# Enderdead/Pytorch_Quantize_impls

Hardware: AMD Instinct MI355X
Metric: XNOR-popcount GEMM TOPS (LinearBin 4096x4096 forward, batch 4096 per GPU) (higher is better)
Workload: dtype fp4-e2m1 (+-1 exact) MFMA, fp32 accumulate, fp32 in/out; 1 GPU; c2: LinearBin(4096, 4096).train().forward(x) on fp32 +-1 activations = sign+pack(x) + sign+pack(W) + packed GEMM, timed through the module (autograd node included); batch_per_gpu=4096, in_features=4096, out_features=4096, global_batch=4096, parallelism=batch-shard x1, no collective, gemm_impl=mfma, detect_mode=verify, float_split=f16x2

## Files before the change

include/qt_hip.h:

```cpp
#ifndef QT_HIP_H
#define QT_HIP_H

#include <stdint.h>

#ifdef __cplusplus
extern "C" {
#endif

typedef void* qt_stream_t;

typedef enum qt_status {
    QT_OK = 0,
    QT_ERR_INVALID_ARG = -1,
    QT_ERR_ALIGNMENT = -2,
    QT_ERR_LAUNCH = -3,
    QT_ERR_UNSUPPORTED = -4,
    QT_ERR_NO_DEVICE = -5
} qt_status;

int qt_version(void);
const char* qt_strerror(int status);
const char* qt_target_arch(void);
int qt_device_info(char* name, int cap);

// ... 82 lines not shown
int qt_tern_gemm(const uint32_t* Xs, int64_t ldxp, const uint32_t* Wmask, const uint32_t* Wsign,
                 int64_t ldwp, const float* bias, float* Y, int64_t ldy, int64_t M, int64_t N,
                 int64_t K, qt_stream_t stream);


int qt_sign_pack_nib_f32(const float* x, int64_t ldx, uint32_t* nib_plane, int64_t ldp,
                         int64_t rows, int64_t K, qt_stream_t stream);

int qt_ternary_pack_nib_f32(const float* x, int64_t ldx, uint32_t* nib_plane, int64_t ldp,
                            int64_t rows, int64_t K, qt_stream_t stream);

int qt_sign0_pack_nib_f32(const float* x, int64_t ldx, uint32_t* nib_plane, int64_t ldp, int64_t rows, int64_t K,
                          qt_stream_t stream);

int qt_pack_pair_nib_f32(const float* x, int64_t ldx, uint32_t* x_plane, int64_t ldxp, int64_t rows_x,
                         const float* w, int64_t ldw, uint32_t* w_plane, int64_t ldwp, int64_t rows_w,
                         int64_t K, int w_ternary, qt_stream_t stream);

int qt_nib_gemm_describe(int64_t M, int64_t N, int64_t K, int64_t ldxp, int64_t ldwp, char* out, int cap);

int qt_nib_gemm(const uint32_t* Xn, int64_t ldxp, const uint32_t* Wn, int64_t ldwp,
                const float* bias, float* Y, int64_t ldy, int64_t M, int64_t N, int64_t K,
                qt_stream_t stream);


int qt_dorefa_codes_i8(const float* x, int64_t ldx, int8_t* codes, int64_t ldc_bytes, float* y_f32,
                       int64_t ldy, int64_t rows, int64_t K, int bit_width, int32_t* overflow,
                       qt_stream_t stream);

int qt_bn_eval_device_f32(const float* x, int64_t ldx, const float* weight, const float* bias, const float* bn_stats, float* y,
                          int64_t ldy, int64_t rows, int64_t C, qt_stream_t stream);

int qt_affine_dorefa_codes_i8(const float* x, int64_t ldx, const float* alpha, const float* beta,
                              const float* res_f32, int64_t ldr, const float* res_alpha, const float* res_beta,
                              const int8_t* res_codes, int64_t ldrc_bytes, float res_scale, int relu, int8_t* codes,
                              int64_t ldc_bytes, float* y_f32, int64_t ldy, int64_t rows, int64_t C, int bit_width,
                              int32_t* overflow, const float* bn_stats, const float* res_bn_stats, qt_stream_t stream);

int qt_affine_dorefa_codes_halo_i8(const float* x, int64_t ldx, const float* alpha, const float* beta,
                                   const float* res_f32, int64_t ldr, const float* res_alpha, const float* res_beta,
                                   const int8_t* res_codes, int64_t ldrc_bytes, float res_scale, int relu, int8_t* codes,
                                   int64_t ldc_bytes, int64_t N, int64_t H, int64_t W, int64_t C, int bit_width,
                                   int32_t* overflow, const float* bn_stats, const float* res_bn_stats, int64_t out_halo_h,
                                   int64_t out_halo_w, qt_stream_t stream);

int qt_codes_to_f32(const int8_t* codes, int64_t ld_bytes, int64_t N, int64_t H, int64_t W, int64_t halo_h, int64_t halo_w,
// ... 257 lines not shown
```

pytorch_quantize_impls_amd/_lib.py:

```python
from __future__ import annotations

import ctypes
import os
import re
import threading
from collections import Counter

_HERE = os.path.dirname(os.path.abspath(__file__))
LIB_PATH = os.environ.get("QT_HIP_LIB") or os.path.join(_HERE, "lib", "libqt_hip.so")
HEADER_PATH = os.path.normpath(os.path.join(_HERE, "..", "include", "qt_hip.h"))


class QtLibraryError(RuntimeError):
    """libqt_hip.so could not be loaded (not built, wrong arch, missing symbol)."""


class QtStatusError(RuntimeError):
    """A C-ABI entry point returned a negative qt_status."""


_c_i64 = ctypes.c_int64
_c_p = ctypes.c_void_p
_c_int = ctypes.c_int
_c_f32 = ctypes.c_float
# ... 39 lines not shown
    "qt_ternary_pack_nib_f32": (_c_int, [_c_p, _c_i64, _c_p, _c_i64, _c_i64, _c_i64, _c_p]),
    "qt_sign0_pack_nib_f32": (_c_int, [_c_p, _c_i64, _c_p, _c_i64, _c_i64, _c_i64, _c_p]),
    "qt_pack_pair_nib_f32": (_c_int, [_c_p, _c_i64, _c_p, _c_i64, _c_i64, _c_p, _c_i64, _c_p, _c_i64, _c_i64, _c_i64,
                                      _c_int, _c_p]),
    "qt_wgrad_pack_grad_f32": (_c_int, [_c_p, _c_i64, _c_i64, _c_i64, _c_i64, _c_i64, _c_i64, _c_i64, _c_i64, _c_i64, _c_p,
                                        _c_i64, _c_p]),
    "qt_wgrad_pack_act_f32": (_c_int, [_c_p, _c_i64, _c_i64, _c_i64, _c_i64, _c_i64, _c_i64, _c_i64, _c_i64, _c_i64, _c_i64,
                                       _c_i64, _c_i64, _c_f32, _c_p, _c_i64, _c_i64, _c_p]),
    "qt_bf16_gemm_taps": (_c_int, [_c_p, _c_i64, _c_p, _c_i64, _c_p, _c_i64, _c_i64, _c_i64, _c_i64, _c_i64, _c_i64, _c_i64,
                                   _c_i64, _c_i64, _c_i64, _c_p]),
    "qt_wgrad_reduce_f32": (_c_int, [_c_p, _c_i64, _c_i64, _c_i64, _c_i64, _c_i64, _c_i64, _c_p, _c_f32, _c_f32, _c_int, _c_p,
                                     _c_p]),
    "qt_wgrad_pm_pack_grad_f32": (_c_int, [_c_p] + [_c_i64] * 11 + [_c_p, _c_p]),
    "qt_wgrad_pm_pack_grad_bias_f32": (_c_int, [_c_p] + [_c_i64] * 10 + [_c_p, _c_p, _c_p]),
    "qt_wgrad_pm_bias_reduce_f32": (_c_int, [_c_p, _c_i64, _c_i64, _c_i64, _c_int, _c_p, _c_p]),
    "qt_wgrad_pm_pack_act_f32": (_c_int, [_c_p] + [_c_i64] * 13 + [_c_f32, _c_p, _c_p]),
    "qt_wgrad_pm_pack_act_s2d_f32": (_c_int, [_c_p] + [_c_i64] * 17 + [_c_p, _c_p]),
    "qt_wgrad_pm_pack_act_s2d_f16x2": (_c_int, [_c_p] + [_c_i64] * 17 + [_c_p, _c_p, _c_p]),
    "qt_wgrad_pm_pack_grad_f16x2": (_c_int, [_c_p] + [_c_i64] * 11 + [_c_p, _c_p, _c_p, _c_p]),
    "qt_wgrad_pm_pack_act_f16": (_c_int, [_c_p] + [_c_i64] * 13 + [_c_f32, _c_p, _c_p]),
    "qt_wgrad_pm_f16": (_c_int, [_c_p, _c_p, _c_p] + [_c_i64] * 7 + [_c_p]),
    "qt_wgrad_pm_f32": (_c_int, [_c_p, _c_p, _c_p] + [_c_i64] * 7 + [_c_p]),
    "qt_wgrad_pm_reduce_f32": (_c_int, [_c_p] + [_c_i64] * 6 + [_c_p, _c_f32, _c_f32, _c_p, _c_int, _c_p] + [_c_i64] * 4 + [_c_p]),
    "qt_nib_gemm_describe": (_c_int, [_c_i64, _c_i64, _c_i64, _c_i64, _c_i64, ctypes.c_char_p, _c_int]),
    "qt_nib_gemm": (_c_int, [_c_p, _c_i64, _c_p, _c_i64, _c_p, _c_p, _c_i64, _c_i64, _c_i64,
                             _c_i64, _c_p]),
    "qt_bits_to_nib": (_c_int, [_c_p, _c_p, _c_i64, _c_p, _c_i64, _c_i64, _c_i64, _c_p]),
    "qt_pack_conv_weight_codes_i8": (_c_int, [_c_p] + [_c_i64] * 8 + [_c_int, _c_p, _c_i64, _c_p]),
    "qt_dorefa_codes_i8": (_c_int, [_c_p, _c_i64, _c_p, _c_i64, _c_p, _c_i64, _c_i64, _c_i64, _c_int, _c_p, _c_p]),
    "qt_bn_eval_device_f32": (_c_int, [_c_p, _c_i64, _c_p, _c_p, _c_p, _c_p, _c_i64, _c_i64, _c_i64, _c_p]),
    "qt_affine_dorefa_codes_i8": (_c_int, [_c_p, _c_i64, _c_p, _c_p, _c_p, _c_i64, _c_p, _c_p, _c_p, _c_i64, _c_f32,
                                           _c_int, _c_p, _c_i64, _c_p, _c_i64, _c_i64, _c_i64, _c_int, _c_p, _c_p, _c_p, _c_p]),
    "qt_affine_dorefa_codes_halo_i8": (_c_int, [_c_p, _c_i64, _c_p, _c_p, _c_p, _c_i64, _c_p, _c_p, _c_p, _c_i64, _c_f32,
                                                _c_int, _c_p, _c_i64, _c_i64, _c_i64, _c_i64, _c_i64, _c_int, _c_p, _c_p, _c_p,
                                                _c_i64, _c_i64, _c_p]),
    "qt_codes_to_f32": (_c_int, [_c_p] + [_c_i64] * 7 + [_c_f32, _c_p, _c_i64, _c_p, _c_i64, _c_p]),
    "qt_weight_codes_i8": (_c_int, [_c_p, _c_i64, _c_p, _c_i64, _c_i64, _c_i64, _c_int, _c_p]),
    "qt_i8_gemm": (_c_int, [_c_p, _c_i64, _c_p, _c_i64, _c_p, _c_f32, _c_p, _c_i64, _c_p, _c_i64, _c_i64,
                            _c_i64, _c_i64, _c_p]),
    "qt_pool_affine_sign_pack_nhwc": (_c_int, [_c_p, _c_i64, _c_i64, _c_i64, _c_i64, _c_i64, _c_i64, _c_p, _c_p,
                                               _c_p, _c_i64, _c_int, _c_p]),
    "qt_pool_affine_sign_pack_nib_nhwc": (_c_int, [_c_p, _c_i64, _c_i64, _c_i64, _c_i64, _c_i64, _c_i64, _c_p, _c_p,
                                                   _c_p, _c_i64, _c_p, _c_i64, _c_int, _c_p]),
    "qt_bf16x3_pack_f32": (_c_int, [_c_p, _c_i64, _c_p, _c_p, _c_i64, _c_i64, _c_i64, _c_int, _c_p]),
    "qt_bf16x3_s2d_pack_f32": (_c_int, [_c_p, _c_i64, _c_i64, _c_i64, _c_i64, _c_p, _c_i64] + [_c_i64] * 7 + [_c_p]),
    "qt_bf16x6_pack_f32": (_c_int, [_c_p, _c_i64, _c_p, _c_i64, _c_i64, _c_i64, _c_int, _c_p]),
# ... 142 lines not shown
```

pytorch_quantize_impls_amd/csrc/mfma_gemm.hip:

```cpp

#include <cstdio>
#include "mfma_gemm_kernel.h"

namespace {

int check_common(const void* Xn, int64_t ldxp, const void* Wn, int64_t ldwp, const float* Y, int64_t ldy,
                 int64_t M, int64_t N, int64_t K, int64_t kwords) {
    if (M < 0 || N < 0 || K < 0) return QT_ERR_INVALID_ARG;
    if (M == 0 || N == 0) return 1;
    if (!Y || ldy < N) return QT_ERR_INVALID_ARG;
    if (M > INT32_MAX || N > INT32_MAX || K > INT32_MAX) return QT_ERR_UNSUPPORTED;
    if (K > 0 && (!Xn || !Wn)) return QT_ERR_INVALID_ARG;
    if (ldxp < kwords || ldwp < kwords) return QT_ERR_INVALID_ARG;
    if ((ldxp & 3) || (ldwp & 3)) return QT_ERR_ALIGNMENT;
    if (K > 0 && (!qt_aligned16(Xn) || !qt_aligned16(Wn))) return QT_ERR_ALIGNMENT;
    return QT_OK;
}

template <class E>
int dispatch_gemm(int variant, const uint32_t* Xn, int64_t ldxp, const uint32_t* Wn, int64_t ldwp,
                  const float* bias, float scale, const float* scale_dev, float* Y, int64_t ldy, int64_t M,
                  int64_t N, int64_t K, qt_stream_t stream) {
    const bool pipe_ok = !(ldxp & 31) && !(ldwp & 31) && M * ldxp * 4 < (1ll << 31) &&
                         N * ldwp * 4 < (1ll << 31);
// ... 82 lines not shown
                                                            uint32_t* __restrict__ oa, int64_t ldpa, int64_t rowsa,
                                                            const float* __restrict__ xb, int64_t ldb,
                                                            uint32_t* __restrict__ ob, int64_t ldpb, int64_t rowsb,
                                                            int64_t K) {
    const int64_t ta = rowsa * ldpa * 2, total = ta + rowsb * ldpb * 2;
    const int64_t k4 = K / 4;
    for (int64_t s = (int64_t)blockIdx.x * blockDim.x + threadIdx.x; s < total;
         s += (int64_t)gridDim.x * blockDim.x) {
        const bool second = s >= ta;
        const int64_t t = second ? s - ta : s;
        const int64_t spr = (second ? ldpb : ldpa) * 2;
        const int64_t row = t / spr, slot = t - row * spr;
        uint32_t h = 0;
        if (slot < k4) {
            const float4 v = *reinterpret_cast<const float4*>((second ? xb + row * ldb : xa + row * lda) + slot * 4);
            h = second ? (EncW::nib(v.x) | (EncW::nib(v.y) << 4) | (EncW::nib(v.z) << 8) | (EncW::nib(v.w) << 12))
                       : (NibSign::nib(v.x) | (NibSign::nib(v.y) << 4) | (NibSign::nib(v.z) << 8) | (NibSign::nib(v.w) << 12));
        }
        const uint32_t other = __shfl_xor(h, 1);
        if ((threadIdx.x & 1) == 0) (second ? ob + row * ldpb : oa + row * ldpa)[slot >> 1] = h | (other << 16);
    }
}

template <class Enc>
__global__ __launch_bounds__(256) void nib_pack_scalar_kernel(const float* __restrict__ x, int64_t ldx,
                                                              uint32_t* __restrict__ out, int64_t ldp,
                                                              int64_t rows, int64_t K) {
    const int64_t total = rows * ldp;
    for (int64_t i = (int64_t)blockIdx.x * blockDim.x + threadIdx.x; i < total;
         i += (int64_t)gridDim.x * blockDim.x) {
        const int64_t row = i / ldp, w = i - row * ldp;
        uint32_t word = 0;
#pragma unroll
        for (int e = 0; e < 8; ++e) {
            const int64_t k = w * 8 + e;
            if (k < K) word |= Enc::nib(x[row * ldx + k]) << (4 * e);
        }
        out[i] = word;
    }
}

__global__ __launch_bounds__(256) void bits_to_nib_kernel(const uint32_t* __restrict__ sign,
                                                          const uint32_t* __restrict__ mask,
                                                          int64_t ldb, uint32_t* __restrict__ out,
                                                          int64_t ldn, int64_t rows, int64_t K) {
    const int64_t groups_per_row = ldn / 4;
// ... 108 lines not shown
                         int w_ternary, qt_stream_t stream) {
    if (rows_x < 0 || rows_w < 0 || K < 0 || ldx < K || ldw < K) return QT_ERR_INVALID_ARG;
    const bool vec = rows_x > 0 && rows_w > 0 && K > 0 && (K % 4 == 0) && (ldx % 4 == 0) && (ldw % 4 == 0) &&
                     qt_aligned16(x) && qt_aligned16(w) && x && w && x_plane && w_plane;
    if (!vec) {
        const int rc = launch_nib_pack<NibSign>(x, ldx, x_plane, ldxp, rows_x, K, stream);
        if (rc != QT_OK) return rc;
        return w_ternary ? launch_nib_pack<NibTernary>(w, ldw, w_plane, ldwp, rows_w, K, stream)
                         : launch_nib_pack<NibSign>(w, ldw, w_plane, ldwp, rows_w, K, stream);
    }
    const int64_t kw = (K + 7) / 8;
    if (ldxp < kw || ldwp < kw || (ldxp & 3) || (ldwp & 3) || !qt_aligned16(x_plane) || !qt_aligned16(w_plane))
        return QT_ERR_ALIGNMENT;
    const int grid = qt_stream_grid(((rows_x * ldxp + rows_w * ldwp) * 2 + 255) / 256);
    if (w_ternary)
        hipLaunchKernelGGL((nib_pack_pair_kernel<NibTernary>), dim3(grid), dim3(256), 0, (hipStream_t)stream, x, ldx,
                           x_plane, ldxp, rows_x, w, ldw, w_plane, ldwp, rows_w, K);
    else
        hipLaunchKernelGGL((nib_pack_pair_kernel<NibSign>), dim3(grid), dim3(256), 0, (hipStream_t)stream, x, ldx,
                           x_plane, ldxp, rows_x, w, ldw, w_plane, ldwp, rows_w, K);
    return qt_check_launch();
}

int qt_nib_gemm_variant(int variant, const uint32_t* Xn, int64_t ldxp, const uint32_t* Wn,
                        int64_t ldwp, const float* bias, float* Y, int64_t ldy, int64_t M, int64_t N,
                        int64_t K, qt_stream_t stream) {
    const int rc = check_common(Xn, ldxp, Wn, ldwp, Y, ldy, M, N, K, (K + 7) / 8);
    if (rc != QT_OK) return rc > 0 ? QT_OK : rc;
    if (K >= (1 << 24)) return QT_ERR_UNSUPPORTED;
    return dispatch_gemm<ElemFp4>(variant, Xn, ldxp, Wn, ldwp, bias, 1.0f, nullptr, Y, ldy, M, N, K, stream);
}

int qt_nib_gemm_describe(int64_t M, int64_t N, int64_t K, int64_t ldxp, int64_t ldwp, char* out, int cap) {
    if (!out || cap < 2 || M <= 0 || N <= 0 || K < 0) return QT_ERR_INVALID_ARG;
    const bool pipe_ok = !(ldxp & 31) && !(ldwp & 31) && M * ldxp * 4 < (1ll << 31) && N * ldwp * 4 < (1ll << 31);
    const int tn = pick_tile_n_gemm(M, N);
    const char* cfg;
    if (pipe_ok && M <= 256 && !((ldxp | ldwp) & 127)) cfg = "64x64, 512-byte stages, pipe=1";
    else if (pipe_ok && M <= 512 && !((ldxp | ldwp) & 63)) cfg = "128x64, 256-byte stages, pipe=1";
    else if (pipe_ok && tn == 256) cfg = "256x256, pipe=2 (ping-pong)";
    else if (pipe_ok && tn == 192) cfg = prefer_384_rows(M, N) ? "384x192, pipe=2 (ping-pong)" : "256x192, pipe=2 (ping-pong)";
    else if (pipe_ok && tn == 128) cfg = "256x128, pipe=2 (ping-pong)";
    else if (pipe_ok) cfg = "256x64, pipe=1";
    else cfg = tn == 256 ? "256x256, pipe=0" : tn == 192 ? "256x192, pipe=0" : tn == 128 ? "256x128, pipe=0" : "256x64, pipe=0";
    snprintf(out, (size_t)cap, "mfma_gemm_kernel<ElemFp4, %s>", cfg);
    return QT_OK;
}

int qt_nib_gemm(const uint32_t* Xn, int64_t ldxp, const uint32_t* Wn, int64_t ldwp, const float* bias,
                float* Y, int64_t ldy, int64_t M, int64_t N, int64_t K, qt_stream_t stream) {
    return qt_nib_gemm_variant(0, Xn, ldxp, Wn, ldwp, bias, Y, ldy, M, N, K, stream);
}

int qt_bf16_gemm(const uint32_t* Xh, int64_t ldxp, const uint32_t* Wh, int64_t ldwp, const float* bias,
                 float* Y, int64_t ldy, int64_t M, int64_t N, int64_t K, qt_stream_t stream) {
    const int rc = check_common(Xh, ldxp, Wh, ldwp, Y, ldy, M, N, K, (K + 1) / 2);
    if (rc != QT_OK) return rc > 0 ? QT_OK : rc;
    return dispatch_gemm<ElemBf16>(0, Xh, ldxp, Wh, ldwp, bias, 1.0f, nullptr, Y, ldy, M, N, K, stream);
}

int qt_f16_gemm(const uint32_t* Xh, int64_t ldxp, const uint32_t* Wh, int64_t ldwp, const float* bias, float scale,
                const float* scale_dev, float* Y, int64_t ldy, int64_t M, int64_t N, int64_t K, qt_stream_t stream) {
    const int rc = check_common(Xh, ldxp, Wh, ldwp, Y, ldy, M, N, K, (K + 1) / 2);
    if (rc != QT_OK) return rc > 0 ? QT_OK : rc;
    return dispatch_gemm<ElemF16>(0, Xh, ldxp, Wh, ldwp, bias, scale, scale_dev, Y, ldy, M, N, K, stream);
}

int qt_bf16_gemm_taps(const uint32_t* Xh, int64_t ldxp, const uint32_t* Wh, int64_t ldwp, float* Y, int64_t ldy,
                      int64_t M, int64_t N, int64_t K, int64_t tap_rows, int64_t tap_cols, int64_t nslice,
// ... 344 lines not shown
```

pytorch_quantize_impls_amd/csrc/mfma_gemm_kernel.h:

```cpp
#pragma once
#include <cstdlib>
#include <type_traits>
#include "qt_common.h"
#include "pp_common.h"

namespace {

__device__ __attribute__((aligned(16))) const unsigned char zero16_storage[16] = {0};


struct ConvArgs {
    int H, W, Ho, Wo, kh, kw, sh, sw, ph, pw, dh, dw;
    int cpp;
    int kbytes;
    unsigned magic_cpp, magic_kw;
    int sh_hw = -1, sh_w = -1;
    int z_nslice = 0, z_kw = 1;
    long long z_kslice_bytes = 0, z_w_copy_bytes = 0, z_w_row_bytes = 0, z_y_stride = 0;
};

struct EpiArgs {
    const float* alpha = nullptr;
    const float* beta = nullptr;
    int mode = 0;
    int relu = 0;
    float levels = 0.0f;
    float rscale = 0.0f;
    const float* res_f32 = nullptr;
    const float* ralpha = nullptr;
    const float* rbeta = nullptr;
    const int8_t* res_codes = nullptr;
    int64_t ldr = 0, ldrc = 0;
    int32_t* overflow = nullptr;
    int ohy = 0, ohx = 0, rhy = 0, rhx = 0;
    int d2s_cout = 0;
    const float* thr = nullptr;
    const float* bn_stats = nullptr;
    unsigned long long magic_hw = 0, magic_w = 0;
    const float* tap_rho = nullptr;
    int tap_ksteps = 0, ntaps = 0;
    const float* row_A = nullptr;
    int aH = 0, aW = 0, aph = 0, apw = 0;
};

__device__ __forceinline__ uint32_t spread8(uint32_t b) {
    uint32_t t = b & 0xFFu;
    t = (t | (t << 12)) & 0x000F000Fu;
    t = (t | (t << 6)) & 0x03030303u;
    t = (t | (t << 3)) & 0x11111111u;
    return t;
}

__device__ __forceinline__ void zero_halo_border(void* plane, int cpp, int64_t nimg, int H, int W, int hy, int hx,
                                                 int zb, int nzb) {
    const int Hp = H + 2 * hy, Wp = W + 2 * hx;
    const int top = hy * Wp, side = 2 * hx * H, per_img = 2 * top + side;
    const int64_t total = nimg * per_img * cpp;
    uint4* Q = reinterpret_cast<uint4*>(plane);
    for (int64_t t = (int64_t)zb * blockDim.x + threadIdx.x; t < total; t += (int64_t)nzb * blockDim.x) {
        const int64_t bp = t / cpp;
        const int c = (int)(t - bp * cpp);
        const int64_t n = bp / per_img;
        const int b = (int)(bp - n * per_img);
        int pix;
        if (b < top) pix = b;
// ... 54 lines not shown
        typedef _Float16 h8 __attribute__((ext_vector_type(8)));
        h8 av, bv;
        __builtin_memcpy(&av, &a, 16);
        __builtin_memcpy(&bv, &b, 16);
        return __builtin_amdgcn_mfma_f32_32x32x16_f16(av, bv, c, 0, 0, 0);
    }
    __device__ __forceinline__ static float out(float v, float scale, float bias) { return v * scale + bias; }
};

struct ElemFp4Taps : ElemFp4 {
    static constexpr bool TAPS = true;
    __device__ __forceinline__ static float out(float v, float scale, float bias) { return v * scale + bias; }
};
struct ElemF16Taps : ElemF16 {
    static constexpr bool TAPS = true;
};
struct ElemFp4TapsRows : ElemFp4Taps {
    static constexpr bool ROWS = true;
};
struct ElemFp4T : ElemFp4 {
    static constexpr bool SWAPT = true;
    __device__ __forceinline__ static acc_t mfma(const uint4& a, const uint4& b, acc_t c) { return ElemFp4::mfma(b, a, c); }
};
template <class E, class = void> struct elem_swapt : std::false_type {};
template <class E> struct elem_swapt<E, std::void_t<decltype(E::SWAPT)>> : std::bool_constant<E::SWAPT> {};
template <class E, class = void> struct elem_rows : std::false_type {};
template <class E> struct elem_rows<E, std::void_t<decltype(E::ROWS)>> : std::bool_constant<E::ROWS> {};

template <class E_, int WM_, int WN_, int TMW_, int TNW_, int PIPE_, int ABL_ = 0, int SB_ = 128, int CONV_ = 0, int OCC_ = 1>
struct GemmCfg {
    using E = E_;
    static constexpr bool CONV = CONV_ != 0, VALID = CONV_ == 2;
    static constexpr int WM = WM_, WN = WN_, TMW = TMW_, TNW = TNW_, PIPE = PIPE_, ABL = ABL_;
    static constexpr int STAGE_BYTES = SB_, KK = SB_ / 32;
    static constexpr int ROWS_PER_PIECE = 1024 / SB_;
    static constexpr int CHUNKS = SB_ / 16;
    static constexpr int NWAVES = WM * WN, NTHREADS = NWAVES * 64;
    static constexpr int TM = WM * TMW * 32, TN = WN * TNW * 32;
    static constexpr int X_STAGE = TM * STAGE_BYTES, W_STAGE = TN * STAGE_BYTES;
    static constexpr int BUF = X_STAGE + W_STAGE;
    static constexpr int NBUF = PIPE_ == 2 ? 4 : (PIPE_ >= 3 ? PIPE_ : 2);
    static constexpr int LDS_FIXED = NBUF * BUF + 64;
    static constexpr int LDS_BYTES = LDS_FIXED;
    static_assert(PIPE_ != 2 || (SB_ == 64 && NWAVES == 8), "ping-pong: 64-byte stages, two waves per SIMD");
    static constexpr int WAVES_PER_SIMD = OCC_ * ((NWAVES + 3) / 4);
    static_assert(TM % (ROWS_PER_PIECE * NWAVES) == 0 && (TN % (ROWS_PER_PIECE * NWAVES) == 0 || PIPE_ >= 1),
// ... 19 lines not shown
        const int gx = (N + C::TN - 1) / C::TN, gy = (M + C::TM - 1) / C::TM;
        const int ntiles = gx * gy, per_xcd = (ntiles + 7) >> 3;
        const int b = blockIdx.x;
        if constexpr (C::CONV) {
            if (b >= 8 * per_xcd) {
                const int zs = epi.d2s_cout ? 2 : 1;
                zero_halo_border(Y, (int)(epi.mode == 2 ? ldy / 16 : ldy / 4), (int64_t)M / (cg.Ho * cg.Wo), zs * cg.Ho,
                                 zs * cg.Wo, epi.ohy, epi.ohx, b - 8 * per_xcd, (int)gridDim.x - 8 * per_xcd);
                return;
            }
        }
        const int o = (b & 7) * per_xcd + (b >> 3);
        if (o >= ntiles) return;
        if ((gx & 7) == 0 && (gy & 3) == 0) {
            const int st = o >> 5, in_st = o & 31, sgx = gx >> 3;
            tile_m = (st / sgx) * 4 + (in_st >> 3);
            tile_n = (st % sgx) * 8 + (in_st & 7);
        } else {
            tile_m = o / gx;
            tile_n = o - tile_m * gx;
        }
    }
    const int m0 = tile_m * C::TM, n0 = tile_n * C::TN;

    const int64_t ldx_b = ldx * 4, ldw_b = ldw * 4;
    const unsigned char* Xb = reinterpret_cast<const unsigned char*>(X);
    const unsigned char* Wb = reinterpret_cast<const unsigned char*>(W);
    if constexpr (!C::CONV && (std::is_same<E, ElemBf16>::value || std::is_same<E, ElemI8>::value)) {
        if (cg.z_nslice > 0) {
            const int z = blockIdx.y, slice = z / cg.H, tap = z - slice * cg.H;
            const int tr = tap / cg.z_kw, tc = tap - tr * cg.z_kw;
            Xb += (int64_t)slice * cg.z_kslice_bytes;
            Wb += (int64_t)slice * cg.z_kslice_bytes + (int64_t)tc * cg.z_w_copy_bytes + (int64_t)tr * cg.z_w_row_bytes;
            Y += ((int64_t)tap * cg.z_nslice + slice) * cg.z_y_stride;
        }
    }

    acc_t acc[C::TMW][C::TNW];
    constexpr bool SWAPT = elem_swapt<E>::value;
    if constexpr (SWAPT) {
#pragma unroll
        for (int b = 0; b < C::TNW; ++b) {
            const int nb = n0 + (wave_n * C::TNW + b) * 32 + 16 * lhalf;
#pragma unroll
            for (int r4 = 0; r4 < 4; ++r4) {
                float4 t = make_float4(0, 0, 0, 0);
// ... 381 lines not shown
            dma_operand(Xb, ldx_b, m0, M, smem, C::TM, 0);
            dma_operand(Wb, ldw_b, n0, N, smem + C::X_STAGE, C::TN, 0);
        }
        __syncthreads();
        for (int s = 0; s < nstages; ++s) {
            const int buf = s & 1;
            const unsigned char* xs = smem + buf * BUF;
            const unsigned char* ws = xs + C::X_STAGE;
            uint4 xf[KK][C::TMW], wf[KK][C::TNW];
#pragma unroll
            for (int kk = 0; kk < KK; ++kk) read_frags(xs, ws, kk, xf[kk], wf[kk]);
            if (s + 1 < nstages) {
                dma_operand(Xb, ldx_b, m0, M, smem + (buf ^ 1) * BUF, C::TM, s + 1);
                dma_operand(Wb, ldw_b, n0, N, smem + (buf ^ 1) * BUF + C::X_STAGE, C::TN, s + 1);
            }
#pragma unroll
            for (int kk = 0; kk < KK; ++kk) mfma_step(xf[kk], wf[kk]);
            __builtin_amdgcn_sched_barrier(0);
            __syncthreads();
        }
    }

    if (scale_dev) scale *= *scale_dev;
    if constexpr (E::TAPS) scale *= epi.tap_rho[epi.ntaps];
    if constexpr (elem_rows<E>::value) {
        const float* ft = ftab + 4 * lhalf;
#pragma unroll
        for (int a = 0; a < C::TMW; ++a) {
#pragma unroll
            for (int j = 0; j < 4; ++j) {
                const float4 f4 = *reinterpret_cast<const float4*>(ft + (wave_m * C::TMW + a) * 32 + 8 * j);
#pragma unroll
                for (int b = 0; b < C::TNW; ++b) {
                    acc[a][b][4 * j + 0] *= f4.x;
                    acc[a][b][4 * j + 1] *= f4.y;
                    acc[a][b][4 * j + 2] *= f4.z;
                    acc[a][b][4 * j + 3] *= f4.w;
                }
            }
        }
        __syncthreads();
    }
    const bool wide = ((ldy & 3) == 0) && ((N & 3) == 0) && ((reinterpret_cast<uintptr_t>(Y) & 15) == 0);
    if constexpr (SWAPT) {
        uint32_t* B = reinterpret_cast<uint32_t*>(Y);
        uint32_t negw[C::TNW], nn[C::TNW][2];
// ... 444 lines not shown
        asm volatile("s_waitcnt vmcnt(0)" ::: "memory");
        dbg_wall[4] = wall_clock64();
        if (lane == 0 && wave_n == 0) {
            unsigned long long* o = reinterpret_cast<unsigned long long*>(Y + (int64_t)(m0 + wave_m * C::TMW * 32) * ldy + n0);
            for (int i = 0; i < 8; ++i) o[i] = dbg_ts[i];
            o[8] = dbg_end;
            for (int i = 0; i < 5; ++i) o[9 + i] = dbg_wall[i];
            o[14] = (unsigned long long)dbg_simd;
            o[15] = dbg_end - dbg_loop0;
        }
    }
}

template <class C>
int launch_cfg(const uint32_t* Xn, int64_t ldxp, const uint32_t* Wn, int64_t ldwp, const float* bias,
               float scale, const float* scale_dev, float* Y, int64_t ldy, int64_t M, int64_t N, int64_t K,
               qt_stream_t stream, const ConvArgs& cg = ConvArgs{}, const EpiArgs& epi = EpiArgs{}) {
    const int64_t gy = (M + C::TM - 1) / C::TM, gx = (N + C::TN - 1) / C::TN;
    if (gx * gy > (1ll << 30)) return QT_ERR_UNSUPPORTED;
    unsigned grid = (unsigned)((gx * gy + 7) / 8 * 8);
    if (C::CONV && (epi.mode == 2 || epi.mode == 3) && (epi.ohy | epi.ohx)) grid += 64;
    const int lds_bytes = C::LDS_BYTES + (C::VALID ? ((cg.kbytes + C::STAGE_BYTES - 1) / C::STAGE_BYTES) * C::CHUNKS * 4 : 0) +
                          (C::E::TAPS ? (epi.ntaps + 1 + 3) / 4 * 16 : 0) +
                          (elem_rows<typename C::E>::value ? (epi.ntaps + 1) * C::TM * 4 : 0);
    if (lds_bytes > 160 * 1024) return QT_ERR_UNSUPPORTED;
    if constexpr (C::E::CODE_EPI && C::CONV) {
        if ((epi.mode == 2 || epi.mode == 4) && epi.bn_stats) {
            static QtLdsOnce once_bn;
            if (qt_ensure_dyn_lds(once_bn, reinterpret_cast<const void*>(mfma_gemm_kernel<C, true>), lds_bytes) != QT_OK) return QT_ERR_LAUNCH;
            hipLaunchKernelGGL((mfma_gemm_kernel<C, true>), dim3(grid, 1), dim3(C::NTHREADS), lds_bytes, (hipStream_t)stream, Xn,
                               ldxp, Wn, ldwp, bias, scale, scale_dev, Y, ldy, (int)M, (int)N, (int)K, cg, epi);
            return qt_check_launch();
        }
    }
    static QtLdsOnce once;
    if (qt_ensure_dyn_lds(once, reinterpret_cast<const void*>(mfma_gemm_kernel<C>), lds_bytes) != QT_OK) return QT_ERR_LAUNCH;
    const unsigned nz = (!C::CONV && cg.z_nslice > 0) ? (unsigned)(cg.z_nslice * cg.H) : 1u;
    hipLaunchKernelGGL(mfma_gemm_kernel<C>, dim3(grid, nz), dim3(C::NTHREADS),
                       lds_bytes, (hipStream_t)stream, Xn, ldxp, Wn, ldwp, bias, scale, scale_dev, Y, ldy,
                       (int)M, (int)N, (int)K, cg, epi);
    return qt_check_launch();
}

template <class E, int PIPE, int ABL = 0> using Cfg256 = GemmCfg<E, 2, 4, 4, 2, PIPE, ABL>;
template <class E, int PIPE> using Cfg128 = GemmCfg<E, 2, 4, 4, 1, PIPE>;
template <class E, int PIPE> using Cfg64 = GemmCfg<E, 4, 2, 2, 1, PIPE>;
template <class E, int PIPE> using Cfg192 = GemmCfg<E, 4, 2, 2, 3, PIPE>;
// ... 130 lines not shown
```

pytorch_quantize_impls_amd/functions/_fused.py:

```python
from __future__ import annotations

import contextlib
import threading
import weakref
from collections import Counter
from typing import Optional

import torch
import torch.nn.functional as F

from .. import ops, packed
from .common import QtFunction

DETECT_BINARY_INPUT = True


LIBRARY_PATHS: Counter = Counter()


_SCOPED = ("GEMM_IMPL", "DETECT_BINARY_INPUT", "FLOAT_PATH", "PAD_PLANES", "XNOR_LINEAR_DIGITS", "BWD_CONV_MFMA", "LINEAR_GRAD_X_ONE_PACK",
           "BWD_MFMA_MIN_MACS")
_scope_tls = threading.local()


# ... 196 lines not shown
        ok, flag = detect_pm1(input, weight)
        if not ok:
            return None, None
    return ops.pack_activations(input, impl), flag


def quant_linear_forward(input: torch.Tensor, weight: torch.Tensor, bias: Optional[torch.Tensor],
                         kind: str, weight_q: Optional[torch.Tensor] = None,
                         weight_planes: Optional[ops.BitPlanes] = None,
                         binary_input: Optional[bool] = None) -> torch.Tensor:
    if not input.is_cuda:
        wq = weight_q if weight_q is not None else quantize_weight_f32(weight, kind)
        return F.linear(input, wq, bias)

    K = input.shape[-1]
    N = weight.shape[0]
    M = input.numel() // max(K, 1)
    impl = ops.select_gemm_impl(_cfg("GEMM_IMPL"), M, N, K)
    if (impl == "mfma" and weight_planes is None and input.dtype == torch.float32 and input.numel() > 0
            and binary_input is not False and packed.lookup(input, packed.ROWS_LAST) is None):
        ok, flag = (True, None) if binary_input else (detect_pm1(input, weight) if _cfg("DETECT_BINARY_INPUT") else (False, None))
        if ok:
            wq = weight_q if weight_q is not None else weight
            xp, wp = ops.pack_linear_operands(input, wq.reshape(N, -1), kind, impl)
            return ops.packed_gemm(xp, wp, poison_bias(bias, flag, N, input.device), impl=impl).view(*input.shape[:-1], N)
        binary_input = False
    xp, flag = activation_planes(input, binary_input, impl, weight)
    if xp is not None:
        wp = weight_planes
        if wp is None:
            wq = weight_q if weight_q is not None else weight
            wp = pack_weight(wq.reshape(N, -1), kind, impl)
        y = ops.packed_gemm(xp, wp, poison_bias(bias, flag, N, input.device), impl=impl)
        return y.view(*input.shape[:-1], N)

    if _cfg("FLOAT_PATH") == "bf16x3" and input.dtype == torch.float32 and input.numel() > 0:
        return ops.float_linear(input, weight_q if weight_q is not None else weight, kind, bias,
                                weight_triples=weight_planes if isinstance(weight_planes, ops.TriplePlanes) else None)
    wq = weight_q if weight_q is not None else quantize_weight_f32(weight, kind)
    note_library_path(input, "non-fp32 or empty linear input")
    return F.linear(input, wq, bias)


def _pixel_planes(input: torch.Tensor, binary_input: Optional[bool], weight: Optional[torch.Tensor] = None, ld_fn=None):
    if input.dtype != torch.float32 or input.dim() != 4 or input.numel() == 0:
        return None, None
# ... 1076 lines not shown
```

pytorch_quantize_impls_amd/ops.py:

```python
from __future__ import annotations

import contextlib
import threading
import functools
from dataclasses import dataclass
from typing import Optional, Tuple

import torch

from . import _lib

STE_THRESHOLD = 1.001

IM2COL_MAX_BYTES = 1 << 30

CONV_IMPLICIT = True

_SCOPED = ("FIRST_DIRECT", "CONV_IMPLICIT", "POPC_VARIANT", "CONV_VARIANT", "ASSUME_CODES_FIT", "PAD_PIXEL_PLANES", "FIRST_3X3", "DIRECT_BITS_128")
_scope_tls = threading.local()


def _cfg(name: str):
    ov = getattr(_scope_tls, "ov", None)
    if ov is not None and name in ov:
# ... 2675 lines not shown
    raise NotImplementedError(impl)


def pack_linear_operands(x: torch.Tensor, w: torch.Tensor, kind: str = "binary", impl: str = "valu"):
    if impl != "mfma":
        return pack_activations(x, impl), pack_weights(w, kind, impl)
    _require(x, "input")
    _require(w, "weight")
    x2, w2 = _as_rows(x), _as_rows(w.reshape(w.shape[0], -1))
    (M, K), (N, Kw) = (int(v) for v in x2.shape), (int(v) for v in w2.shape)
    if K != Kw:
        raise ValueError(f"K mismatch: activations {K} vs weights {Kw}")
    ld = packed_ld_nib(K)
    xn = torch.empty((M, ld), dtype=torch.int32, device=x.device)
    wn = torch.empty((N, ld), dtype=torch.int32, device=x.device)
    I = int
    with _on(x.device):
        _lib.call("qt_pack_pair_nib_f32", _p(x2), I(x2.stride(0) if M > 1 else max(K, 1)), _p(xn), I(ld), I(M),
                  _p(w2), I(w2.stride(0) if N > 1 else max(K, 1)), _p(wn), I(ld), I(N), I(K),
                  int(0 if kind == "binary" else 1), _stream(x.device))
    return NibPlanes(words=xn, rows=M, K=K), NibPlanes(words=wn, rows=N, K=K)


def to_impl(planes, impl: str):
    if impl == "valu":
        if isinstance(planes, BitPlanes):
            return planes
        raise TypeError("nibble planes cannot feed the popcount GEMM")
    if isinstance(planes, NibPlanes):
        return planes
    if getattr(planes, "nib", None) is not None:
        return planes.nib
    return bits_to_nib(planes)


def packed_gemm(x, w, bias=None, out=None, impl: str = "valu") -> torch.Tensor:
    if impl == "valu":
        return tern_gemm(x, w, bias, out) if w.is_ternary else xnor_gemm(x, w, bias, out)
    if impl == "mfma":
        return nib_gemm(to_impl(x, "mfma"), to_impl(w, "mfma"), bias, out)
    raise NotImplementedError(impl)


def nib_gemm_kernel_name(M: int, N: int, K: int) -> str:
    import ctypes
    buf = ctypes.create_string_buffer(128)
# ... 13 lines not shown
```

Measured before the change: 2295 TOPS.

## Add 0/1 fp4 encoding path with count-corrected epilogue for binary linear

Measured after the change: 2416 TOPS (median of 6 runs). 1.05x the previous value.

```diff
diff --git a/include/qt_hip.h b/include/qt_hip.h
--- a/include/qt_hip.h
+++ b/include/qt_hip.h
@@ -128,6 +128,16 @@
 int qt_nib_gemm(const uint32_t* Xn, int64_t ldxp, const uint32_t* Wn, int64_t ldwp,
                 const float* bias, float* Y, int64_t ldy, int64_t M, int64_t N, int64_t K,
                 qt_stream_t stream);
+
+int qt_pack_pair_nib01_f32(const float* x, int64_t ldx, uint32_t* x_plane, int64_t ldxp, int32_t* x_count, int64_t rows_x,
+                           const float* w, int64_t ldw, uint32_t* w_plane, int64_t ldwp, int32_t* w_count, int64_t rows_w,
+                           int64_t K, qt_stream_t stream);
+
+int qt_nib01_gemm_supported(int64_t M, int64_t N, int64_t K, int64_t ldxp, int64_t ldwp);
+
+int qt_nib01_gemm(const uint32_t* Xn, int64_t ldxp, const int32_t* x_count, const uint32_t* Wn, int64_t ldwp,
+                  const int32_t* w_count, const float* bias, float* Y, int64_t ldy, int64_t M, int64_t N, int64_t K,
+                  qt_stream_t stream);
 
 
 int qt_dorefa_codes_i8(const float* x, int64_t ldx, int8_t* codes, int64_t ldc_bytes, float* y_f32,
diff --git a/pytorch_quantize_impls_amd/_lib.py b/pytorch_quantize_impls_amd/_lib.py
--- a/pytorch_quantize_impls_amd/_lib.py
+++ b/pytorch_quantize_impls_amd/_lib.py
@@ -85,6 +85,10 @@
     "qt_wgrad_pm_f16": (_c_int, [_c_p, _c_p, _c_p] + [_c_i64] * 7 + [_c_p]),
     "qt_wgrad_pm_f32": (_c_int, [_c_p, _c_p, _c_p] + [_c_i64] * 7 + [_c_p]),
     "qt_wgrad_pm_reduce_f32": (_c_int, [_c_p] + [_c_i64] * 6 + [_c_p, _c_f32, _c_f32, _c_p, _c_int, _c_p] + [_c_i64] * 4 + [_c_p]),
+    "qt_pack_pair_nib01_f32": (_c_int, [_c_p, _c_i64, _c_p, _c_i64, _c_p, _c_i64, _c_p, _c_i64, _c_p, _c_i64, _c_p, _c_i64,
+                                        _c_i64, _c_p]),
+    "qt_nib01_gemm_supported": (_c_int, [_c_i64, _c_i64, _c_i64, _c_i64, _c_i64]),
+    "qt_nib01_gemm": (_c_int, [_c_p, _c_i64, _c_p, _c_p, _c_i64, _c_p, _c_p, _c_p, _c_i64, _c_i64, _c_i64, _c_i64, _c_p]),
     "qt_nib_gemm_describe": (_c_int, [_c_i64, _c_i64, _c_i64, _c_i64, _c_i64, ctypes.c_char_p, _c_int]),
     "qt_nib_gemm": (_c_int, [_c_p, _c_i64, _c_p, _c_i64, _c_p, _c_p, _c_i64, _c_i64, _c_i64,
                              _c_i64, _c_p]),
diff --git a/pytorch_quantize_impls_amd/csrc/mfma_gemm.hip b/pytorch_quantize_impls_amd/csrc/mfma_gemm.hip
--- a/pytorch_quantize_impls_amd/csrc/mfma_gemm.hip
+++ b/pytorch_quantize_impls_amd/csrc/mfma_gemm.hip
@@ -128,6 +128,47 @@
     }
 }
 
+__global__ __launch_bounds__(256) void nib01_pack_pair_kernel(const float* __restrict__ xa, int lda,
+                                                              uint32_t* __restrict__ oa, int ldpa, int rowsa,
+                                                              const float* __restrict__ xb, int ldb,
+                                                              uint32_t* __restrict__ ob, int ldpb, int rowsb,
+                                                              int32_t* __restrict__ ca, int32_t* __restrict__ cb, int K) {
+    __shared__ int wsum[4];
+    const int t = threadIdx.x, lane = t & 63, wave = t >> 6;
+    const int k4 = K >> 2;
+    for (int r = blockIdx.x; r < rowsa + rowsb; r += gridDim.x) {
+        const bool second = r >= rowsa;
+        const int row = second ? r - rowsa : r;
+        const float4* src = reinterpret_cast<const float4*>(second ? xb + (int64_t)row * ldb : xa + (int64_t)row * lda);
+        uint32_t* dst = second ? ob + (int64_t)row * ldpb : oa + (int64_t)row * ldpa;
+        const int spr = (second ? ldpb : ldpa) * 2;
+        int cnt = 0;
+        for (int base = 0; base < spr; base += 1024) {
+            float4 v[4];
+#pragma unroll
+            for (int i = 0; i < 4; ++i) {
+                const int slot = base + i * 256 + t;
+                v[i] = slot < k4 ? src[slot] : make_float4(-1.f, -1.f, -1.f, -1.f);
+            }
+#pragma unroll
+            for (int i = 0; i < 4; ++i) {
+                const uint32_t h = (v[i].x < 0.f ? 0u : 0x2u) | (v[i].y < 0.f ? 0u : 0x20u) |
+                                   (v[i].z < 0.f ? 0u : 0x200u) | (v[i].w < 0.f ? 0u : 0x2000u);
+                cnt += __popc(h);
+                const uint32_t other = __shfl_xor(h, 1);
+                const int slot = base + i * 256 + t;
+                if (!(t & 1) && slot < spr) dst[slot >> 1] = h | (other << 16);
+            }
+        }
+#pragma unroll
+        for (int o = 32; o > 0; o >>= 1) cnt += __shfl_xor(cnt, o);
+        if (lane == 0) wsum[wave] = cnt;
+        __syncthreads();
+        if (t == 0) (second ? cb : ca)[row] = wsum[0] + wsum[1] + wsum[2] + wsum[3];
+        __syncthreads();
+    }
+}
+
 template <class Enc>
 __global__ __launch_bounds__(256) void nib_pack_scalar_kernel(const float* __restrict__ x, int64_t ldx,
                                                               uint32_t* __restrict__ out, int64_t ldp,
@@ -282,6 +323,39 @@
     return qt_check_launch();
 }
 
+int qt_pack_pair_nib01_f32(const float* x, int64_t ldx, uint32_t* x_plane, int64_t ldxp, int32_t* x_count, int64_t rows_x,
+                           const float* w, int64_t ldw, uint32_t* w_plane, int64_t ldwp, int32_t* w_count, int64_t rows_w,
+                           int64_t K, qt_stream_t stream) {
+    if (rows_x < 0 || rows_w < 0 || K < 0 || ldx < K || ldw < K) return QT_ERR_INVALID_ARG;
+    if (rows_x + rows_w == 0) return QT_OK;
+    if ((rows_x && (!x_plane || !x_count || (!x && K))) || (rows_w && (!w_plane || !w_count || (!w && K))))
+        return QT_ERR_INVALID_ARG;
+    const int64_t kw = (K + 7) / 8;
+    if (ldxp < kw || ldwp < kw || (ldxp & 3) || (ldwp & 3) || !qt_aligned16(x_plane) || !qt_aligned16(w_plane))
+        return QT_ERR_ALIGNMENT;
+    if ((K & 3) || (ldx & 3) || (ldw & 3) || !qt_aligned16(x) || !qt_aligned16(w)) return QT_ERR_ALIGNMENT;
+    if (rows_x + rows_w > INT32_MAX || ldx > INT32_MAX || ldw > INT32_MAX || ldxp > (1 << 29) || ldwp > (1 << 29))
+        return QT_ERR_UNSUPPORTED;
+    const int grid = (int)std::min<int64_t>(rows_x + rows_w, 256 * 64);
+    hipLaunchKernelGGL(nib01_pack_pair_kernel, dim3(grid), dim3(256), 0, (hipStream_t)stream, x, (int)ldx, x_plane,
+                       (int)ldxp, (int)rows_x, w, (int)ldw, w_plane, (int)ldwp, (int)rows_w, x_count, w_count, (int)K);
+    return qt_check_launch();
+}
+
+int qt_nib01_gemm(const uint32_t* Xn, int64_t ldxp, const int32_t* x_count, const uint32_t* Wn, int64_t ldwp,
+                  const int32_t* w_count, const float* bias, float* Y, int64_t ldy, int64_t M, int64_t N, int64_t K,
+                  qt_stream_t stream) {
+    const int rc = check_common(Xn, ldxp, Wn, ldwp, Y, ldy, M, N, K, (K + 7) / 8);
+    if (rc != QT_OK) return rc > 0 ? QT_OK : rc;
+    if (!x_count || !w_count) return QT_ERR_INVALID_ARG;
+    if (K >= (1 << 22)) return QT_ERR_UNSUPPORTED;
+    if (qt_nib01_gemm_supported(M, N, K, ldxp, ldwp) != 1) return QT_ERR_UNSUPPORTED;
+    EpiArgs epi;
+    epi.cnt_x = x_count;
+    epi.cnt_w = w_count;
+    return launch_cfg<PP256<ElemFp4U>>(Xn, ldxp, Wn, ldwp, bias, 1.0f, nullptr, Y, ldy, M, N, K, stream, ConvArgs{}, epi);
+}
+
 int qt_nib_gemm_variant(int variant, const uint32_t* Xn, int64_t ldxp, const uint32_t* Wn,
                         int64_t ldwp, const float* bias, float* Y, int64_t ldy, int64_t M, int64_t N,
                         int64_t K, qt_stream_t stream) {
@@ -305,6 +379,15 @@
     else cfg = tn == 256 ? "256x256, pipe=0" : tn == 192 ? "256x192, pipe=0" : tn == 128 ? "256x128, pipe=0" : "256x64, pipe=0";
     snprintf(out, (size_t)cap, "mfma_gemm_kernel<ElemFp4, %s>", cfg);
     return QT_OK;
+}
+
+int qt_nib01_gemm_supported(int64_t M, int64_t N, int64_t K, int64_t ldxp, int64_t ldwp) {
+    if (M <= 0 || N <= 0 || K <= 0 || K >= (1 << 22)) return 0;
+    const bool pipe_ok = !(ldxp & 31) && !(ldwp & 31) && M * ldxp * 4 < (1ll << 31) && N * ldwp * 4 < (1ll << 31);
+    if (!pipe_ok || M > INT32_MAX || N > INT32_MAX) return 0;
+    if ((M <= 256 && !((ldxp | ldwp) & 127)) || (M <= 512 && !((ldxp | ldwp) & 63))) return 0;
+    if (pick_tile_n_gemm(M, N) != 256) return 0;
+    return ((M + 255) / 256) * ((N + 255) / 256) >= 256 ? 1 : 0;
 }
 
 int qt_nib_gemm(const uint32_t* Xn, int64_t ldxp, const uint32_t* Wn, int64_t ldwp, const float* bias,
diff --git a/pytorch_quantize_impls_amd/csrc/mfma_gemm_kernel.h b/pytorch_quantize_impls_amd/csrc/mfma_gemm_kernel.h
--- a/pytorch_quantize_impls_amd/csrc/mfma_gemm_kernel.h
+++ b/pytorch_quantize_impls_amd/csrc/mfma_gemm_kernel.h
@@ -41,6 +41,8 @@
     int tap_ksteps = 0, ntaps = 0;
     const float* row_A = nullptr;
     int aH = 0, aW = 0, aph = 0, apw = 0;
+    const int32_t* cnt_x = nullptr;
+    const int32_t* cnt_w = nullptr;
 };
 
 __device__ __forceinline__ uint32_t spread8(uint32_t b) {
@@ -141,6 +143,11 @@
     static constexpr bool SWAPT = true;
     __device__ __forceinline__ static acc_t mfma(const uint4& a, const uint4& b, acc_t c) { return ElemFp4::mfma(b, a, c); }
 };
+struct ElemFp4U : ElemFp4 {
+    static constexpr bool COUNTS = true;
+};
+template <class E, class = void> struct elem_counts : std::false_type {};
+template <class E> struct elem_counts<E, std::void_t<decltype(E::COUNTS)>> : std::bool_constant<E::COUNTS> {};
 template <class E, class = void> struct elem_swapt : std::false_type {};
 template <class E> struct elem_swapt<E, std::void_t<decltype(E::SWAPT)>> : std::bool_constant<E::SWAPT> {};
 template <class E, class = void> struct elem_rows : std::false_type {};
@@ -206,6 +213,15 @@
         }
     }
     const int m0 = tile_m * C::TM, n0 = tile_n * C::TN;
+    [[maybe_unused]] int cnt_own = 0;
+    if constexpr (elem_counts<E>::value) {
+        static_assert(C::TM + C::TN <= C::NTHREADS && !C::CONV, "one count per thread, GEMM only");
+        if (tid < C::TM) {
+            if (m0 + tid < M) cnt_own = epi.cnt_x[m0 + tid];
+        } else if (tid < C::TM + C::TN) {
+            if (n0 + tid - C::TM < N) cnt_own = epi.cnt_w[n0 + tid - C::TM];
+        }
+    }
 
     const int64_t ldx_b = ldx * 4, ldw_b = ldw * 4;
     const unsigned char* Xb = reinterpret_cast<const unsigned char*>(X);
@@ -633,6 +649,29 @@
     }
 
     if (scale_dev) scale *= *scale_dev;
+    if constexpr (elem_counts<E>::value) {
+        float* ctab = reinterpret_cast<float*>(smem + C::NBUF * BUF + 64);
+        if (tid < C::TM) ctab[tid] = (float)(-2 * cnt_own);
+        else if (tid < C::TM + C::TN) ctab[tid] = (float)(K - 2 * cnt_own);
+        __syncthreads();
+        float cb[C::TNW];
+#pragma unroll
+        for (int b = 0; b < C::TNW; ++b) cb[b] = ctab[C::TM + (wave_n * C::TNW + b) * 32 + lrow];
+#pragma unroll
+        for (int a = 0; a < C::TMW; ++a) {
+#pragma unroll
+            for (int j = 0; j < 4; ++j) {
+                const float4 ca = *reinterpret_cast<const float4*>(ctab + (wave_m * C::TMW + a) * 32 + 4 * lhalf + 8 * j);
+#pragma unroll
+                for (int b = 0; b < C::TNW; ++b) {
+                    acc[a][b][4 * j + 0] = fmaf(acc[a][b][4 * j + 0], 4.0f, ca.x + cb[b]);
+                    acc[a][b][4 * j + 1] = fmaf(acc[a][b][4 * j + 1], 4.0f, ca.y + cb[b]);
+                    acc[a][b][4 * j + 2] = fmaf(acc[a][b][4 * j + 2], 4.0f, ca.z + cb[b]);
+                    acc[a][b][4 * j + 3] = fmaf(acc[a][b][4 * j + 3], 4.0f, ca.w + cb[b]);
+                }
+            }
+        }
+    }
     if constexpr (E::TAPS) scale *= epi.tap_rho[epi.ntaps];
     if constexpr (elem_rows<E>::value) {
         const float* ft = ftab + 4 * lhalf;
@@ -1123,7 +1162,8 @@
     if (C::CONV && (epi.mode == 2 || epi.mode == 3) && (epi.ohy | epi.ohx)) grid += 64;
     const int lds_bytes = C::LDS_BYTES + (C::VALID ? ((cg.kbytes + C::STAGE_BYTES - 1) / C::STAGE_BYTES) * C::CHUNKS * 4 : 0) +
                           (C::E::TAPS ? (epi.ntaps + 1 + 3) / 4 * 16 : 0) +
-                          (elem_rows<typename C::E>::value ? (epi.ntaps + 1) * C::TM * 4 : 0);
+                          (elem_rows<typename C::E>::value ? (epi.ntaps + 1) * C::TM * 4 : 0) +
+                          (elem_counts<typename C::E>::value ? (C::TM + C::TN) * 4 : 0);
     if (lds_bytes > 160 * 1024) return QT_ERR_UNSUPPORTED;
     if constexpr (C::E::CODE_EPI && C::CONV) {
         if ((epi.mode == 2 || epi.mode == 4) && epi.bn_stats) {
diff --git a/pytorch_quantize_impls_amd/functions/_fused.py b/pytorch_quantize_impls_amd/functions/_fused.py
--- a/pytorch_quantize_impls_amd/functions/_fused.py
+++ b/pytorch_quantize_impls_amd/functions/_fused.py
@@ -242,6 +242,10 @@
         ok, flag = (True, None) if binary_input else (detect_pm1(input, weight) if _cfg("DETECT_BINARY_INPUT") else (False, None))
         if ok:
             wq = weight_q if weight_q is not None else weight
+            if (kind == "binary" and wq.dtype == torch.float32 and wq.is_contiguous() and input.is_contiguous()
+                    and ops.nib01_route_ok(M, N, K) and input.data_ptr() % 16 == 0 and wq.data_ptr() % 16 == 0):
+                xu, wu = ops.pack_linear_operands01(input, wq.reshape(N, -1))
+                return ops.nib01_gemm(xu, wu, poison_bias(bias, flag, N, input.device)).view(*input.shape[:-1], N)
             xp, wp = ops.pack_linear_operands(input, wq.reshape(N, -1), kind, impl)
             return ops.packed_gemm(xp, wp, poison_bias(bias, flag, N, input.device), impl=impl).view(*input.shape[:-1], N)
         binary_input = False
diff --git a/pytorch_quantize_impls_amd/ops.py b/pytorch_quantize_impls_amd/ops.py
--- a/pytorch_quantize_impls_amd/ops.py
+++ b/pytorch_quantize_impls_amd/ops.py
@@ -2721,6 +2721,66 @@
     return NibPlanes(words=xn, rows=M, K=K), NibPlanes(words=wn, rows=N, K=K)
 
 
+@dataclass
+class Nib01Planes:
+    words: torch.Tensor
+    count: torch.Tensor
+    rows: int
+    K: int
+
+    @property
+    def ld(self) -> int:
+        return int(self.words.shape[1])
+
+    @property
+    def device(self):
+        return self.words.device
+
+
+@functools.lru_cache(maxsize=256)
+def nib01_route_ok(M: int, N: int, K: int) -> bool:
+    if M <= 0 or N <= 0 or K <= 0 or K % 4:
+        return False
+    ld = packed_ld_nib(K)
+    return _lib.load().qt_nib01_gemm_supported(int(M), int(N), int(K), ld, ld) == 1
+
+
+def pack_linear_operands01(x: torch.Tensor, w: torch.Tensor) -> Tuple[Nib01Planes, Nib01Planes]:
+    _require(x, "input")
+    _require(w, "weight")
+    x2, w2 = _as_rows(x), _as_rows(w.reshape(w.shape[0], -1))
+    (M, K), (N, Kw) = (int(v) for v in x2.shape), (int(v) for v in w2.shape)
+    if K != Kw:
+        raise ValueError(f"K mismatch: activations {K} vs weights {Kw}")
+    ld = packed_ld_nib(K)
+    xn = torch.empty((M, ld), dtype=torch.int32, device=x.device)
+    wn = torch.empty((N, ld), dtype=torch.int32, device=x.device)
+    cnt = torch.empty((M + N,), dtype=torch.int32, device=x.device)
+    I = int
+    with _on(x.device):
+        _lib.call("qt_pack_pair_nib01_f32", _p(x2), I(x2.stride(0) if M > 1 else max(K, 1)), _p(xn), I(ld), _p(cnt), I(M),
+                  _p(w2), I(w2.stride(0) if N > 1 else max(K, 1)), _p(wn), I(ld), _p(cnt[M:]), I(N), I(K),
+                  _stream(x.device))
+    return Nib01Planes(words=xn, count=cnt[:M], rows=M, K=K), Nib01Planes(words=wn, count=cnt[M:], rows=N, K=K)
+
+
+def nib01_gemm(x: Nib01Planes, w: Nib01Planes, bias: Optional[torch.Tensor] = None,
+               out: Optional[torch.Tensor] = None) -> torch.Tensor:
+    if not isinstance(x, Nib01Planes) or not isinstance(w, Nib01Planes):
+        raise TypeError("nib01_gemm takes the Nib01Planes of pack_linear_operands01")
+    if x.K != w.K:
+        raise ValueError(f"K mismatch: activations {x.K} vs weights {w.K}")
+    M, N, K = x.rows, w.rows, x.K
+    dev = x.device
+    bias = _check_bias(bias, N, dev)
+    if out is None:
+        out = torch.empty((M, N), dtype=torch.float32, device=dev)
+    with _on(dev):
+        _lib.call("qt_nib01_gemm", _p(x.words), int(x.ld), _p(x.count), _p(w.words), int(w.ld), _p(w.count), _p(bias),
+                  _p(out), int(out.stride(0) if M > 1 else max(N, 1)), int(M), int(N), int(K), _stream(dev))
+    return out
+
+
 def to_impl(planes, impl: str):
     if impl == "valu":
         if isinstance(planes, BitPlanes):
```
